# jinbeizame007/pytorch-r2d2-DPG

Hardware: NVIDIA H100
Metric: learner sequence-steps/sec (batch x seq_len) (higher is better)
Workload: dtype bf16x3 (fp32 operands split into bf16 hi+lo, three tensor-core passes, fp32 accumulate: ~16-bit operands)

## Files before the change

pytorch-r2d2-dpg_b200/csrc/gemm.cu:

```cuda
#include "gemm.cuh"
#include "elementwise.cuh"

#include <stdlib.h>

namespace r2d2 {
namespace {

constexpr int BM = 128, BN = 64, BK = 32, GEMM_THREADS = 256;

template <int LAYOUT>
struct TileGeom {
  static constexpr bool A_KMAJOR = (LAYOUT != GEMM_TN);
  static constexpr int A_ROWS = A_KMAJOR ? BM : BK;
  static constexpr int A_COLS = A_KMAJOR ? BK : BM;
  static constexpr int A_LD = A_COLS + 8;
  static constexpr bool B_KMAJOR = (LAYOUT == GEMM_NT);
  static constexpr int B_ROWS = B_KMAJOR ? BN : BK;
  static constexpr int B_COLS = B_KMAJOR ? BK : BN;
  static constexpr int B_LD = B_COLS + 8;
  static constexpr int A_PLANE = A_ROWS * A_LD;
  static constexpr int B_PLANE = B_ROWS * B_LD;
  static constexpr int STAGE = 2 * A_PLANE + 2 * B_PLANE;
  static constexpr int SMEM_BYTES = 2 * STAGE * (int)sizeof(__nv_bfloat16);
  static constexpr int A_F4_PER_ROW = A_COLS / 4;
  static constexpr int B_F4_PER_ROW = B_COLS / 4;
  static constexpr int A_F4 = A_ROWS * A_COLS / 4 / GEMM_THREADS;
  static constexpr int B_F4 = B_ROWS * B_COLS / 4 / GEMM_THREADS;
};

__device__ __forceinline__ float4 guarded_load4(const float* __restrict__ base, long long ld, int row, int col,
                                                int row_lim, int col_lim, bool vec) {
  float4 v = make_float4(0.f, 0.f, 0.f, 0.f);
  if (row < row_lim && col < col_lim) {
    const float* p = base + (long long)row * ld + col;
    if (vec && col + 3 < col_lim) {
      v = __ldg(reinterpret_cast<const float4*>(p));
    } else {
      v.x = __ldg(p);
      if (col + 1 < col_lim) v.y = __ldg(p + 1);
      if (col + 2 < col_lim) v.z = __ldg(p + 2);
      if (col + 3 < col_lim) v.w = __ldg(p + 3);
    }
  }
  return v;
}

__device__ __forceinline__ void store_split4(__nv_bfloat16* hi_plane, __nv_bfloat16* lo_plane, int off, float4 v) {
  uint32_t h0, l0, h1, l1;
  split_pack2(v.x, v.y, h0, l0);
  split_pack2(v.z, v.w, h1, l1);
  *reinterpret_cast<uint2*>(hi_plane + off) = make_uint2(h0, h1);
  *reinterpret_cast<uint2*>(lo_plane + off) = make_uint2(l0, l1);
}

template <int LAYOUT>
__global__ void __launch_bounds__(GEMM_THREADS)
gemm_bf16x3_kernel(GemmParams p, int vecA, int vecB, int vecA2, int vecB2, long long c_split_stride) {
  using G = TileGeom<LAYOUT>;
  extern __shared__ __align__(16) unsigned char smem_raw[];
  __nv_bfloat16* smem = reinterpret_cast<__nv_bfloat16*>(smem_raw);

  const int tid = threadIdx.x, lane = tid & 31, warp = tid >> 5;
  const int wm = warp & 3, wn = warp >> 2;
  const int m0 = blockIdx.y * BM, n0 = blockIdx.x * BN;

  const int nk1 = (p.K + BK - 1) / BK;
  const int nk2 = (p.K2 + BK - 1) / BK;
  const int nk_total = nk1 + nk2;
  const int per_split = (nk_total + p.split_k - 1) / p.split_k;
  const int t_begin = blockIdx.z * per_split;
  const int t_end = min(nk_total, t_begin + per_split);
  if (t_begin >= t_end) return;

  float acc[2][4][4];
#pragma unroll
  for (int i = 0; i < 2; ++i)
#pragma unroll
    for (int j = 0; j < 4; ++j)
#pragma unroll
      for (int e = 0; e < 4; ++e) acc[i][j][e] = 0.f;

  float4 ra[G::A_F4], rb[G::B_F4];

  auto load_tile = [&](int t) {
    const float* Ap; const float* Bp; long long lda, ldb; int k0, klim; bool va, vb;
    if (t < nk1) { Ap = p.A; Bp = p.B; lda = p.lda; ldb = p.ldb; k0 = t * BK; klim = p.K; va = vecA; vb = vecB; }
    else { Ap = p.A2; Bp = p.B2; lda = p.lda2; ldb = p.ldb2; k0 = (t - nk1) * BK; klim = p.K2; va = vecA2; vb = vecB2; }
#pragma unroll
    for (int i = 0; i < G::A_F4; ++i) {
      int q = tid + i * GEMM_THREADS;
      int r = q / G::A_F4_PER_ROW, c = (q % G::A_F4_PER_ROW) * 4;
      if (G::A_KMAJOR) ra[i] = guarded_load4(Ap, lda, m0 + r, k0 + c, p.M, klim, va);
      else             ra[i] = guarded_load4(Ap, lda, k0 + r, m0 + c, klim, p.M, va);
    }
#pragma unroll
    for (int i = 0; i < G::B_F4; ++i) {
      int q = tid + i * GEMM_THREADS;
      int r = q / G::B_F4_PER_ROW, c = (q % G::B_F4_PER_ROW) * 4;
      if (G::B_KMAJOR) rb[i] = guarded_load4(Bp, ldb, n0 + r, k0 + c, p.N, klim, vb);
      else             rb[i] = guarded_load4(Bp, ldb, k0 + r, n0 + c, klim, p.N, vb);
    }
  };

  auto store_tile = [&](int buf) {
    __nv_bfloat16* a_hi = smem + buf * G::STAGE;
    __nv_bfloat16* a_lo = a_hi + G::A_PLANE;
    __nv_bfloat16* b_hi = a_lo + G::A_PLANE;
    __nv_bfloat16* b_lo = b_hi + G::B_PLANE;
#pragma unroll
    for (int i = 0; i < G::A_F4; ++i) {
      int q = tid + i * GEMM_THREADS;
      int r = q / G::A_F4_PER_ROW, c = (q % G::A_F4_PER_ROW) * 4;
      store_split4(a_hi, a_lo, r * G::A_LD + c, ra[i]);
    }
#pragma unroll
    for (int i = 0; i < G::B_F4; ++i) {
      int q = tid + i * GEMM_THREADS;
      int r = q / G::B_F4_PER_ROW, c = (q % G::B_F4_PER_ROW) * 4;
      store_split4(b_hi, b_lo, r * G::B_LD + c, rb[i]);
    }
  };

  auto compute_tile = [&](int buf) {
    const __nv_bfloat16* a_hi = smem + buf * G::STAGE;
    const __nv_bfloat16* a_lo = a_hi + G::A_PLANE;
    const __nv_bfloat16* b_hi = a_lo + G::A_PLANE;
    const __nv_bfloat16* b_lo = b_hi + G::B_PLANE;
    const int j = lane >> 3, r = lane & 7;
#pragma unroll
    for (int kk = 0; kk < BK; kk += 16) {
      uint32_t fa_hi[2][4], fa_lo[2][4], fb_hi[4][2], fb_lo[4][2];
#pragma unroll
      for (int i = 0; i < 2; ++i) {
        if (G::A_KMAJOR) {
          int off = (wm * 32 + i * 16 + (j & 1) * 8 + r) * G::A_LD + kk + (j >> 1) * 8;
          ldmatrix_x4(fa_hi[i], a_hi + off);
          ldmatrix_x4(fa_lo[i], a_lo + off);
        } else {
          int off = (kk + (j >> 1) * 8 + r) * G::A_LD + wm * 32 + i * 16 + (j & 1) * 8;
          ldmatrix_x4_trans(fa_hi[i], a_hi + off);
          ldmatrix_x4_trans(fa_lo[i], a_lo + off);
        }
      }
#pragma unroll
      for (int pj = 0; pj < 2; ++pj) {
        uint32_t th[4], tl[4];
        if (G::B_KMAJOR) {
          int off = (wn * 32 + pj * 16 + (j >> 1) * 8 + r) * G::B_LD + kk + (j & 1) * 8;
          ldmatrix_x4(th, b_hi + off);
          ldmatrix_x4(tl, b_lo + off);
        } else {
          int off = (kk + (j & 1) * 8 + r) * G::B_LD + wn * 32 + pj * 16 + (j >> 1) * 8;
          ldmatrix_x4_trans(th, b_hi + off);
          ldmatrix_x4_trans(tl, b_lo + off);
        }
        fb_hi[2 * pj][0] = th[0]; fb_hi[2 * pj][1] = th[1]; fb_hi[2 * pj + 1][0] = th[2]; fb_hi[2 * pj + 1][1] = th[3];
        fb_lo[2 * pj][0] = tl[0]; fb_lo[2 * pj][1] = tl[1]; fb_lo[2 * pj + 1][0] = tl[2]; fb_lo[2 * pj + 1][1] = tl[3];
      }
#pragma unroll
      for (int i = 0; i < 2; ++i)
#pragma unroll
        for (int jn = 0; jn < 4; ++jn) {
          mma_bf16_16816(acc[i][jn], fa_lo[i], fb_hi[jn]);
          mma_bf16_16816(acc[i][jn], fa_hi[i], fb_lo[jn]);
          mma_bf16_16816(acc[i][jn], fa_hi[i], fb_hi[jn]);
        }
    }
  };

  load_tile(t_begin);
  store_tile(0);
  __syncthreads();
  for (int t = t_begin; t < t_end; ++t) {
    const int buf = (t - t_begin) & 1;
    if (t + 1 < t_end) load_tile(t + 1);
    compute_tile(buf);
    if (t + 1 < t_end) store_tile(buf ^ 1);
    __syncthreads();
  }

  const int g = lane >> 2, c = lane & 3;
  float* const C = p.C + (long long)blockIdx.z * c_split_stride;
  const bool vec_c = ((reinterpret_cast<uintptr_t>(C) & 7) == 0) && (p.ldc % 2 == 0);
#pragma unroll
  for (int i = 0; i < 2; ++i) {
#pragma unroll
    for (int jn = 0; jn < 4; ++jn) {
      const int col = n0 + wn * 32 + jn * 8 + 2 * c;
#pragma unroll
      for (int h = 0; h < 2; ++h) {
        const int row = m0 + wm * 32 + i * 16 + g + h * 8;
        if (row >= p.M || col >= p.N) continue;
        float v0 = acc[i][jn][2 * h], v1 = acc[i][jn][2 * h + 1];
        const bool has1 = (col + 1 < p.N);
        if (p.bias) { v0 += __ldg(p.bias + col); if (has1) v1 += __ldg(p.bias + col + 1); }
        if (p.epilogue == EPI_TANH) { v0 = tanhf(v0); v1 = tanhf(v1); }
        else if (p.epilogue == EPI_MUL_DTANH) {
          const float* z = p.Z + (long long)row * p.ldz + col;
          float z0 = z[0]; v0 *= (1.f - z0 * z0);
          if (has1) { float z1 = z[1]; v1 *= (1.f - z1 * z1); }
        } else if (p.epilogue == EPI_ADD_Z) {
          const float* z = p.Z + (long long)row * p.ldz + col;
          v0 += z[0];
          if (has1) v1 += z[1];
        }
        float* cp = C + (long long)row * p.ldc + col;
        if (vec_c && has1) {
          *reinterpret_cast<float2*>(cp) = make_float2(v0, v1);
        } else {
          cp[0] = v0;
          if (has1) cp[1] = v1;
        }
      }
    }
  }
}

template <int LAYOUT>
int launch_gemm(const GemmParams& p, cudaStream_t stream) {
  using G = TileGeom<LAYOUT>;
  static PerDeviceOnce once;
  if (once.need()) {
    R2D2_CUDA_TRY(cudaFuncSetAttribute(gemm_bf16x3_kernel<LAYOUT>, cudaFuncAttributeMaxDynamicSharedMemorySize,
                                       G::SMEM_BYTES));
  }
  auto aligned = [](const float* ptr, long long ld) {
    return ptr != nullptr && ((reinterpret_cast<uintptr_t>(ptr) & 15) == 0) && (ld % 4 == 0);
  };
  GemmParams q = p;
  int slices = 1;
  if (p.split_k > 1) {
    const int nk = ceil_div(p.K, BK) + ceil_div(p.K2, BK), per_split = ceil_div(nk, p.split_k);
    slices = ceil_div(nk, per_split);
    R2D2_TRY(partials_scratch((size_t)slices * p.M * p.N, stream, &q.C));
    q.ldc = p.N;
  }
  dim3 grid(ceil_div(p.N, BN), ceil_div(p.M, BM), slices);
  gemm_bf16x3_kernel<LAYOUT><<<grid, GEMM_THREADS, G::SMEM_BYTES, stream>>>(
      q, aligned(p.A, p.lda), aligned(p.B, p.ldb), aligned(p.A2, p.lda2), aligned(p.B2, p.ldb2), (long long)p.M * p.N);
  count_launch();
  R2D2_CUDA_TRY(cudaGetLastError());
  if (p.split_k > 1) return add_partials(q.C, slices, p.M, p.N, p.C, p.ldc, nullptr, stream);
  return R2D2_OK;
}

}

static int g_gemm_impl = -1;
void gemm_set_impl(int impl) { g_gemm_impl = impl ? 1 : 0; }
int gemm_get_impl() {
  if (g_gemm_impl < 0) {
    const char* e = getenv("R2D2_GEMM_IMPL");
    g_gemm_impl = (e && (e[0] == 'm' || e[0] == '0')) ? 0 : 1;
  }
  return g_gemm_impl;
}

static int g_skinny_mma = 1;
void gemm_set_impl_skinny_mma(int on) { g_skinny_mma = on ? 1 : 0; }
int gemm_get_impl_skinny_mma() { return g_skinny_mma; }

bool gemm_supports_bias2(int M, int N, int K) {
  const bool skinny = (K < 64) || (N < 32) || (M < 32);
  return gemm_get_impl() == 1 && !(skinny && gemm_get_impl_skinny_mma());
}

bool gemm_emits_operand_image(int M, int N, int K_total) {
  if (gemm_get_impl() != 1 || N <= 32 || N % 32 != 0) return false;
  if (gemm_get_impl_skinny_mma() && K_total <= 32) return true;
  const bool skinny = (K_total < 64) || (M < 32);
  return !(skinny && gemm_get_impl_skinny_mma());
}

int gemm_suggest_split_k(int M, int N, int K) {
  const bool skinny = (K < 64) || (N < 32) || (M < 32);
  if (gemm_get_impl() == 1 && !(skinny && g_skinny_mma)) return gemm_tc_suggest_split_k(M, N, K);
  long long tiles = (long long)ceil_div(M, BM) * ceil_div(N, BN);
  int k_tiles = ceil_div(K, BK);
  if (tiles >= num_sms() || k_tiles < 16) return 1;
  int want = (int)ceil_div_ll(2 * num_sms(), tiles);
  int max_by_k = k_tiles / 8;
  int s = want < max_by_k ? want : max_by_k;
  if (s < 1) s = 1;
  if (s > 128) s = 128;
  return s;
}

static int gemm_f32_dispatch(const GemmParams& p, GemmLayout layout, cudaStream_t stream, bool* colsums_done);

int gemm_f32(const GemmParams& p, GemmLayout layout, cudaStream_t stream) {
  R2D2_REQUIRE((!p.colsum_a && !p.colsum_b) || layout == GEMM_TN, "column sums ride on TN products only");
  bool colsums_done = false;
  R2D2_TRY(gemm_f32_dispatch(p, layout, stream, &colsums_done));
  if (!colsums_done) {
    if (p.colsum_a) R2D2_TRY(colsum(p.A, p.lda, p.K, p.M, p.colsum_a, nullptr, stream));
    if (p.colsum_b) R2D2_TRY(colsum(p.B, p.ldb, p.K, p.N, p.colsum_b, nullptr, stream));
  }
  return R2D2_OK;
}

static int gemm_f32_dispatch(const GemmParams& p, GemmLayout layout, cudaStream_t stream, bool* colsums_done) {
  R2D2_REQUIRE((p.A || p.A_img) && (p.B || p.B_img) && p.C, "null operand");
  if (p.A_img || p.B_img) {
    R2D2_REQUIRE(p.K2 == 0, "packed A with a second K segment");
    return gemm_f32_tc(p, layout, stream);
  }
  R2D2_REQUIRE(p.M > 0 && p.N > 0 && p.K > 0, "empty problem");
  R2D2_REQUIRE(p.split_k >= 1, "split_k");
  R2D2_REQUIRE(p.split_k == 1 || (p.epilogue == EPI_NONE && p.bias == nullptr), "split-K supports no epilogue");
  R2D2_REQUIRE(p.K2 == 0 || layout == GEMM_NT, "second K segment only for NT");
  R2D2_REQUIRE(p.K2 == 0 || (p.A2 && p.B2), "segment 2 operands");
  R2D2_REQUIRE((p.epilogue != EPI_MUL_DTANH && p.epilogue != EPI_ADD_Z) || p.Z, "epilogue needs Z");
  R2D2_REQUIRE(ceil_div(p.M, BM) <= 65535, "M too large for grid.y");
  const bool skinny = (p.K + p.K2 < 64) || (p.N < 32) || (p.M < 32);
  if (gemm_get_impl() == 1 && gemm_get_impl_skinny_mma()) {
    bool handled = false;
    R2D2_TRY(gemm_thin_try(p, layout, stream, &handled));
    if (handled) { *colsums_done = true; return R2D2_OK; }
  }
  R2D2_REQUIRE(!p.bias2 || gemm_supports_bias2(p.M, p.N, p.K + p.K2), "bias2 needs the wgmma path (gemm_supports_bias2)");
  R2D2_REQUIRE((!p.C_img_k && !p.C_img_mn) || (layout == GEMM_NT && gemm_emits_operand_image(p.M, p.N, p.K + p.K2)),
               "C_img_* is produced by the small-K streaming kernel and the wgmma epilogue only (see gemm_emits_operand_image)");
  if (gemm_get_impl() == 1 && !(skinny && gemm_get_impl_skinny_mma())) return gemm_f32_tc(p, layout, stream);
  switch (layout) {
    case GEMM_NT: return launch_gemm<GEMM_NT>(p, stream);
    case GEMM_NN: return launch_gemm<GEMM_NN>(p, stream);
    case GEMM_TN: return launch_gemm<GEMM_TN>(p, stream);
  }
  set_last_error("bad gemm layout");
  return R2D2_ERR_ARG;
}

}
```

pytorch-r2d2-dpg_b200/csrc/gemm.cuh:

```cuda
#pragma once
#include "common.cuh"

namespace r2d2 {

enum GemmLayout : int {
  GEMM_NT = 0,
  GEMM_NN = 1,
  GEMM_TN = 2
};

enum GemmEpilogue : int {
  EPI_NONE = 0,
  EPI_TANH = 1,
  EPI_MUL_DTANH = 2,
  EPI_ADD_Z = 3
};

struct GemmParams {
  const float* A = nullptr;  long long lda = 0;
  const float* B = nullptr;  long long ldb = 0;
  const float* A2 = nullptr; long long lda2 = 0;
  const float* B2 = nullptr; long long ldb2 = 0;
  int K2 = 0;
  float* C = nullptr;        long long ldc = 0;
  int M = 0, N = 0, K = 0;
  const float* bias = nullptr;
  const float* bias2 = nullptr;
  const float* Z = nullptr;  long long ldz = 0;
  int epilogue = EPI_NONE;
  int split_k = 1;
  const unsigned char* A_img = nullptr;
  unsigned char* C_img_k = nullptr;
  unsigned char* C_img_mn = nullptr;
  const unsigned char* B_img = nullptr;
  float* colsum_a = nullptr;
  float* colsum_b = nullptr;
  int reuse_packed_a = 0;
};

int gemm_f32(const GemmParams& p, GemmLayout layout, cudaStream_t stream);
bool gemm_emits_operand_image(int M, int N, int K_total);
bool gemm_supports_bias2(int M, int N, int K);
int gemm_suggest_split_k(int M, int N, int K);

void gemm_set_impl(int impl);
int gemm_get_impl();
void gemm_set_impl_skinny_mma(int on);
int gemm_get_impl_skinny_mma();
int gemm_f32_tc(const GemmParams& p, GemmLayout layout, cudaStream_t stream);
int gemm_thin_try(const GemmParams& p, GemmLayout layout, cudaStream_t stream, bool* handled);
int gemm_tc_suggest_split_k(int M, int N, int K);

}
```

pytorch-r2d2-dpg_b200/csrc/gemm_tc.cu:

```cuda
#include <stdlib.h>

#include <map>
#include <mutex>
#include <utility>

#include "elementwise.cuh"
#include "gemm.cuh"
#include "sm90.cuh"

namespace r2d2 {
namespace {

constexpr int TBM = 128, TBN = 128, TBK = 32;
constexpr int PLANE_BYTES = 128 * TBK * 2;
constexpr int TILE_BYTES = 2 * PLANE_BYTES;
constexpr int PACKED_GEMM_THREADS = 288;
constexpr int CTAS_PER_SM = 2;
constexpr int STAGES = 3;
constexpr int STAGE_BYTES = 2 * TILE_BYTES;
constexpr int OFF_BARS = STAGES * STAGE_BYTES;
constexpr int PACKED_SMEM = OFF_BARS + 128;

template <bool MN_MAJOR>
__global__ void __launch_bounds__(256) pack_operand_kernel(const float* __restrict__ src, long long ld, int mn_lim,
                                                           int k_lim, int k_tiles_total, int k_tile_offset, int vec,
                                                           unsigned char* __restrict__ dst) {
  const int mn0 = blockIdx.y * 128, k0 = blockIdx.x * TBK;
  unsigned char* tile = dst + ((size_t)blockIdx.y * k_tiles_total + k_tile_offset + blockIdx.x) * TILE_BYTES;
#pragma unroll
  for (int g = 0; g < 2; ++g) {
    const int id = threadIdx.x + g * 256;
    int row, col, row_lim, col_lim;
    if (MN_MAJOR) { row = k0 + 8 * (id >> 7) + (id & 7); col = mn0 + 8 * ((id >> 3) & 15); row_lim = k_lim; col_lim = mn_lim; }
    else          { row = mn0 + 8 * (id >> 5) + (id & 7); col = k0 + 8 * ((id >> 3) & 3);  row_lim = mn_lim; col_lim = k_lim; }
    float v[8];
#pragma unroll
    for (int i = 0; i < 8; ++i) v[i] = 0.f;
    if (row < row_lim && col < col_lim) {
      const float* p = src + (long long)row * ld + col;
      if (vec && col + 7 < col_lim) {
        const float4 a = __ldg(reinterpret_cast<const float4*>(p)), b = __ldg(reinterpret_cast<const float4*>(p + 4));
        v[0] = a.x; v[1] = a.y; v[2] = a.z; v[3] = a.w; v[4] = b.x; v[5] = b.y; v[6] = b.z; v[7] = b.w;
      } else {
#pragma unroll
        for (int i = 0; i < 8; ++i) if (col + i < col_lim) v[i] = __ldg(p + i);
      }
    }
    uint4 h, l;
    split_pack2(v[0], v[1], h.x, l.x);
    split_pack2(v[2], v[3], h.y, l.y);
    split_pack2(v[4], v[5], h.z, l.z);
    split_pack2(v[6], v[7], h.w, l.w);
    *reinterpret_cast<uint4*>(tile + id * 16) = h;
    *reinterpret_cast<uint4*>(tile + PLANE_BYTES + id * 16) = l;
  }
}

__device__ __forceinline__ void mbar_wait_spin(uint64_t* bar, uint32_t parity) {
  while (!sm90::mbar_try_wait(bar, parity)) {}
}

struct PackedGemmParams {
  const unsigned char* pa;
  const unsigned char* pb;
  int k_tiles;
  float* C; long long ldc;
  int M, N;
  const float* bias;
  const float* bias2;
  const float* Z; long long ldz;
  int epilogue, split_k;
  long long c_split_stride;
  unsigned char* c_img_k;
  unsigned char* c_img_mn;
};

template <bool A_MN, bool B_MN>
__global__ void __launch_bounds__(PACKED_GEMM_THREADS, CTAS_PER_SM) gemm_packed_kernel(PackedGemmParams p) {
  extern __shared__ __align__(128) unsigned char smem[];
  uint64_t* full = reinterpret_cast<uint64_t*>(smem + OFF_BARS);
  uint64_t* empty = full + STAGES;

  const int tid = threadIdx.x, lane = tid & 31;
  const int wg = __shfl_sync(0xffffffffu, tid >> 7, 0);
  const int m_tile = blockIdx.y, n_tile = blockIdx.x;
  const int m0 = m_tile * TBM, n0 = n_tile * TBN;
  const int per_split = (p.k_tiles + p.split_k - 1) / p.split_k;
  const int t_begin = blockIdx.z * per_split;
  const int t_end = min(p.k_tiles, t_begin + per_split);
  if (t_begin >= t_end) return;
  const int n_tiles = t_end - t_begin;

  if (tid == 0) {
    for (int s = 0; s < STAGES; ++s) { sm90::mbar_init(&full[s], 1); sm90::mbar_init(&empty[s], 2); }
    asm volatile("fence.mbarrier_init.release.cluster;" ::: "memory");
  }
  __syncthreads();

  if (wg == 2) {
    if (sm90::elect_one()) {
      const unsigned char* a_src = p.pa + ((size_t)m_tile * p.k_tiles + t_begin) * TILE_BYTES;
      const unsigned char* b_src = p.pb + ((size_t)n_tile * p.k_tiles + t_begin) * TILE_BYTES;
      const uint32_t smem_base = sm90::smem_u32(smem);
      for (int i = 0; i < n_tiles; ++i) {
        const int s = i % STAGES;
        mbar_wait_spin(&empty[s], ((i / STAGES) & 1) ^ 1);
        const uint32_t bar = sm90::smem_u32(&full[s]);
        sm90::mbar_arrive_expect_tx(&full[s], 2 * TILE_BYTES);
        sm90::bulk_copy_g2s(smem_base + s * STAGE_BYTES, a_src + (size_t)i * TILE_BYTES, TILE_BYTES, bar);
        sm90::bulk_copy_g2s(smem_base + s * STAGE_BYTES + TILE_BYTES, b_src + (size_t)i * TILE_BYTES, TILE_BYTES, bar);
      }
    }
    return;
  }

  const int half = wg, t = tid & 127;
  float acc[64];
#pragma unroll
  for (int i = 0; i < 64; ++i) acc[i] = 0.f;
  const uint32_t a_lbo = A_MN ? 2048 : 128, a_sbo = A_MN ? 128 : 512;
  const uint32_t b_lbo = B_MN ? 2048 : 128, b_sbo = B_MN ? 128 : 512;
  const uint32_t a_ks = A_MN ? 4096 : 256, b_ks = B_MN ? 4096 : 256;
  const uint32_t a_half = half * 8 * a_sbo;
  const uint32_t smem_base = sm90::smem_u32(smem);
  for (int i = 0; i < n_tiles; ++i) {
    const int s = i % STAGES;
    mbar_wait_spin(&full[s], (i / STAGES) & 1);
    const uint32_t sa = smem_base + s * STAGE_BYTES + a_half, sb = smem_base + s * STAGE_BYTES + TILE_BYTES;
    sm90::fence_regs(acc);
    sm90::wgmma_fence();
#pragma unroll
    for (int ks = 0; ks < TBK / 16; ++ks) {
      const uint64_t a_hi = sm90::make_smem_desc(sa + ks * a_ks, a_lbo, a_sbo);
      const uint64_t a_lo = sm90::make_smem_desc(sa + ks * a_ks + PLANE_BYTES, a_lbo, a_sbo);
      const uint64_t b_hi = sm90::make_smem_desc(sb + ks * b_ks, b_lbo, b_sbo);
      const uint64_t b_lo = sm90::make_smem_desc(sb + ks * b_ks + PLANE_BYTES, b_lbo, b_sbo);
      sm90::wgmma_m64n128k16_bf16<A_MN, B_MN>(acc, a_lo, b_hi);
      sm90::wgmma_m64n128k16_bf16<A_MN, B_MN>(acc, a_hi, b_lo);
      sm90::wgmma_m64n128k16_bf16<A_MN, B_MN>(acc, a_hi, b_hi);
    }
    sm90::wgmma_commit();
    sm90::wgmma_wait<1>();
    sm90::fence_regs(acc);
    __syncwarp();
    if (i > 0 && t == 0) sm90::mbar_arrive(&empty[(i - 1) % STAGES]);
  }
  sm90::wgmma_wait<0>();
  sm90::fence_regs(acc);
  __syncwarp();
  if (t == 0) sm90::mbar_arrive(&empty[(n_tiles - 1) % STAGES]);

  const int r_base = m0 + half * 64 + 16 * (t >> 5) + (lane >> 2);
  const int c_off = 2 * (lane & 3);
  float* const C = p.C + (long long)blockIdx.z * p.c_split_stride;
  const bool vec_c = ((reinterpret_cast<uintptr_t>(C) & 7) == 0) && (p.ldc % 2 == 0);
  const bool img = p.c_img_k != nullptr || p.c_img_mn != nullptr;
#pragma unroll
  for (int j = 0; j < TBN / 8; ++j) {
    const int col = n0 + 8 * j + c_off;
    const bool c0ok = col < p.N, c1ok = col + 1 < p.N;
    float b0 = 0.f, b1 = 0.f;
    if (p.bias) {
      if (c0ok) b0 = __ldg(p.bias + col) + (p.bias2 ? __ldg(p.bias2 + col) : 0.f);
      if (c1ok) b1 = __ldg(p.bias + col + 1) + (p.bias2 ? __ldg(p.bias2 + col + 1) : 0.f);
    }
#pragma unroll
    for (int h = 0; h < 2; ++h) {
      const int row = r_base + 8 * h;
      float v0 = acc[4 * j + 2 * h] + b0, v1 = acc[4 * j + 2 * h + 1] + b1;
      if (img) {
        const bool ok = row < p.M && c0ok;
        if (ok) {
          if (p.epilogue == EPI_TANH) { v0 = tanhf(v0); v1 = tanhf(v1); }
          *reinterpret_cast<float2*>(p.C + (long long)row * p.ldc + col) = make_float2(v0, v1);
        } else {
          v0 = v1 = 0.f;
        }
        uint32_t hw, lw;
        split_pack2(v0, v1, hw, lw);
        const int q0 = lane & ~3;
        const uint4 hi = make_uint4(__shfl_sync(0xffffffffu, hw, q0), __shfl_sync(0xffffffffu, hw, q0 + 1),
                                    __shfl_sync(0xffffffffu, hw, q0 + 2), __shfl_sync(0xffffffffu, hw, q0 + 3));
        const uint4 lo = make_uint4(__shfl_sync(0xffffffffu, lw, q0), __shfl_sync(0xffffffffu, lw, q0 + 1),
                                    __shfl_sync(0xffffffffu, lw, q0 + 2), __shfl_sync(0xffffffffu, lw, q0 + 3));
        const int cg = n0 + 8 * j;
        if ((lane & 3) == 0 && cg < p.N && row < ((p.M + 31) & ~31)) {
          if (p.c_img_k && row < p.M) {
            unsigned char* d = p.c_img_k + ((size_t)(row >> 7) * (p.N >> 5) + (cg >> 5)) * TILE_BYTES +
                               ((((row & 127) >> 3) * 32) + ((cg & 31) >> 3) * 8 + (row & 7)) * 16;
            *reinterpret_cast<uint4*>(d) = hi;
            *reinterpret_cast<uint4*>(d + PLANE_BYTES) = lo;
          }
          if (p.c_img_mn) {
            unsigned char* d = p.c_img_mn + ((size_t)(cg >> 7) * ((p.M + 31) >> 5) + (row >> 5)) * TILE_BYTES +
                               ((((row & 31) >> 3) * 128) + ((cg & 127) >> 3) * 8 + (row & 7)) * 16;
            *reinterpret_cast<uint4*>(d) = hi;
            *reinterpret_cast<uint4*>(d + PLANE_BYTES) = lo;
          }
        }
        continue;
      }
      if (row >= p.M || !c0ok) continue;
      if (p.epilogue == EPI_TANH) {
        v0 = tanhf(v0); v1 = tanhf(v1);
      } else if (p.epilogue == EPI_MUL_DTANH || p.epilogue == EPI_ADD_Z) {
        const float* z = p.Z + (long long)row * p.ldz + col;
        const float z0 = z[0], z1 = c1ok ? z[1] : 0.f;
        if (p.epilogue == EPI_MUL_DTANH) { v0 *= 1.f - z0 * z0; v1 *= 1.f - z1 * z1; }
        else { v0 += z0; v1 += z1; }
      }
      float* cp = C + (long long)row * p.ldc + col;
      if (vec_c && c1ok) {
        *reinterpret_cast<float2*>(cp) = make_float2(v0, v1);
      } else {
        cp[0] = v0;
        if (c1ok) cp[1] = v1;
      }
    }
  }
}

struct Scratch { unsigned char* ptr = nullptr; size_t bytes = 0; };
struct LastPackedA { const float* ptr = nullptr; long long ld = 0; int mn = 0, k = 0, mn_major = 0, k_tiles = 0; };
struct StreamScratch { Scratch a, b; LastPackedA last_a; };
std::mutex g_scratch_mutex;
std::map<std::pair<int, cudaStream_t>, StreamScratch> g_scratch;

int scratch_for(cudaStream_t stream, StreamScratch** out) {
  int dev = 0;
  R2D2_CUDA_TRY(cudaGetDevice(&dev));
  std::lock_guard<std::mutex> lock(g_scratch_mutex);
  *out = &g_scratch[std::make_pair(dev, stream)];
  return R2D2_OK;
}

int ensure_scratch(Scratch& s, size_t bytes) {
  if (s.bytes >= bytes) return R2D2_OK;
  if (s.ptr) { R2D2_CUDA_TRY(cudaDeviceSynchronize()); R2D2_CUDA_TRY(cudaFree(s.ptr)); s.ptr = nullptr; s.bytes = 0; }
  const size_t want = bytes + bytes / 4 + (1u << 20);
  R2D2_CUDA_TRY(cudaMalloc(&s.ptr, want));
  s.bytes = want;
  return R2D2_OK;
}

int launch_pack(const float* src, long long ld, int mn_lim, int k_lim, bool mn_major, int mn_tiles, int k_tiles_total,
                int k_tile_offset, unsigned char* dst, cudaStream_t stream) {
  const int vec = (((reinterpret_cast<uintptr_t>(src) & 15) == 0) && (ld % 4 == 0)) ? 1 : 0;
  dim3 grid(ceil_div(k_lim, TBK), mn_tiles);
  if (mn_major) pack_operand_kernel<true><<<grid, 256, 0, stream>>>(src, ld, mn_lim, k_lim, k_tiles_total, k_tile_offset, vec, dst);
  else          pack_operand_kernel<false><<<grid, 256, 0, stream>>>(src, ld, mn_lim, k_lim, k_tiles_total, k_tile_offset, vec, dst);
  count_launch();
  R2D2_CUDA_TRY(cudaGetLastError());
  return R2D2_OK;
}

}

int gemm_tc_suggest_split_k(int M, int N, int K) {
  long long tiles = (long long)ceil_div(M, TBM) * ceil_div(N, TBN);
  int k_tiles = ceil_div(K, TBK);
  if (tiles >= num_sms() || k_tiles < 16) return 1;
  int want = (int)ceil_div_ll(2 * num_sms(), tiles);
  int max_by_k = k_tiles / 8;
  int s = want < max_by_k ? want : max_by_k;
  if (s < 1) s = 1;
  if (s > 256) s = 256;
  return s;
}

template <bool A_MN, bool B_MN>
int launch_packed(const PackedGemmParams& q, int m_tiles, int n_tiles, int slices, cudaStream_t stream) {
  static PerDeviceOnce once;
  if (once.need()) {
    R2D2_CUDA_TRY(cudaFuncSetAttribute(gemm_packed_kernel<A_MN, B_MN>, cudaFuncAttributeMaxDynamicSharedMemorySize,
                                       PACKED_SMEM));
  }
  dim3 grid(n_tiles, m_tiles, slices);
  gemm_packed_kernel<A_MN, B_MN><<<grid, PACKED_GEMM_THREADS, PACKED_SMEM, stream>>>(q);
  count_launch();
  R2D2_CUDA_TRY(cudaGetLastError());
  return R2D2_OK;
}

int gemm_f32_tc(const GemmParams& p, GemmLayout layout, cudaStream_t stream) {
  const bool a_mn = (layout == GEMM_TN), b_mn = (layout != GEMM_NT);
  const int m_tiles = ceil_div(p.M, TBM), n_tiles = ceil_div(p.N, TBN);
  const int kt1 = ceil_div(p.K, TBK), kt2 = p.K2 > 0 ? ceil_div(p.K2, TBK) : 0;
  const int k_tiles = kt1 + kt2;
  R2D2_REQUIRE(m_tiles <= 65535, "M too large for grid.y");
  StreamScratch* sc = nullptr;
  R2D2_TRY(scratch_for(stream, &sc));
  Scratch& g_pack_a = sc->a;
  Scratch& g_pack_b = sc->b;
  LastPackedA& last_a = sc->last_a;
  if (!p.A_img) R2D2_TRY(ensure_scratch(g_pack_a, (size_t)m_tiles * k_tiles * TILE_BYTES));
  if (!p.B_img) R2D2_TRY(ensure_scratch(g_pack_b, (size_t)n_tiles * k_tiles * TILE_BYTES));
  const bool reuse = p.reuse_packed_a && kt2 == 0 && last_a.ptr == p.A && last_a.ld == p.lda && last_a.mn == p.M &&
                     last_a.k == p.K && last_a.mn_major == (a_mn ? 1 : 0) && last_a.k_tiles == k_tiles;
  if (!p.A_img) {
    if (!reuse) R2D2_TRY(launch_pack(p.A, p.lda, p.M, p.K, a_mn, m_tiles, k_tiles, 0, g_pack_a.ptr, stream));
    last_a = LastPackedA{kt2 ? nullptr : p.A, p.lda, p.M, p.K, a_mn ? 1 : 0, k_tiles};
  }
  if (!p.B_img) R2D2_TRY(launch_pack(p.B, p.ldb, p.N, p.K, b_mn, n_tiles, k_tiles, 0, g_pack_b.ptr, stream));
  if (kt2) {
    R2D2_REQUIRE(!p.A_img && !p.B_img, "packed operand with a second K segment");
    R2D2_TRY(launch_pack(p.A2, p.lda2, p.M, p.K2, a_mn, m_tiles, k_tiles, kt1, g_pack_a.ptr, stream));
    R2D2_TRY(launch_pack(p.B2, p.ldb2, p.N, p.K2, b_mn, n_tiles, k_tiles, kt1, g_pack_b.ptr, stream));
  }
  PackedGemmParams q;
  q.pa = p.A_img ? p.A_img : g_pack_a.ptr; q.pb = p.B_img ? p.B_img : g_pack_b.ptr; q.k_tiles = k_tiles; q.C = p.C; q.ldc = p.ldc; q.M = p.M; q.N = p.N;
  q.bias = p.bias; q.bias2 = p.bias ? p.bias2 : nullptr; q.Z = p.Z; q.ldz = p.ldz; q.epilogue = p.epilogue; q.split_k = p.split_k;
  q.c_img_k = p.C_img_k; q.c_img_mn = p.C_img_mn;
  q.c_split_stride = 0;
  int slices = 1;
  if (p.split_k > 1) {
    slices = ceil_div(k_tiles, ceil_div(k_tiles, p.split_k));
    R2D2_TRY(partials_scratch((size_t)slices * p.M * p.N, stream, &q.C));
    q.ldc = p.N;
    q.c_split_stride = (long long)p.M * p.N;
  }
  if (p.C_img_k || p.C_img_mn) {
    R2D2_REQUIRE(p.N % 32 == 0 && p.split_k == 1 && (p.epilogue == EPI_NONE || p.epilogue == EPI_TANH) &&
                     (reinterpret_cast<uintptr_t>(p.C) & 7) == 0 && p.ldc % 2 == 0,
                 "operand image from the wgmma epilogue: N % 32 == 0, no split-K, bias / tanh epilogue, 8-byte aligned C");
  }
  if (a_mn) R2D2_TRY((launch_packed<true, true>(q, m_tiles, n_tiles, slices, stream)));
  else if (b_mn) R2D2_TRY((launch_packed<false, true>(q, m_tiles, n_tiles, slices, stream)));
  else R2D2_TRY((launch_packed<false, false>(q, m_tiles, n_tiles, slices, stream)));
  if (p.split_k > 1) return add_partials(q.C, slices, p.M, p.N, p.C, p.ldc, nullptr, stream);
  return R2D2_OK;
}

}
```

pytorch-r2d2-dpg_b200/csrc/net.cu:

```cuda
#include "net.cuh"

#include "elementwise.cuh"
#include "gemm.cuh"
#include "lstm_scan.cuh"

namespace r2d2 {

static size_t align64(size_t n) { return (n + 63) & ~(size_t)63; }
static size_t pad_to(size_t n, size_t m) { return (n + m - 1) / m * m; }

size_t ChainWs::floats(const NetShape& s, int T, int B, int repeat) {
  const size_t H = s.hidden, A = s.act, S = (size_t)T * repeat, TB = (size_t)T * B;
  size_t n = 0;
  n += align64(TB * H);
  n += align64(TB * 4 * H);
  if (repeat > 1) n += align64(S * B * 4 * H);
  n += 2 * align64((S + 1) * B * H);
  n += align64(TB * H);
  n += align64(TB * H);
  n += 2 * align64(TB * A);
  n += align64(4 * H);
  size_t sc = lstm_scan_fwd_scratch_floats(B, s.hidden);
  const size_t sb = lstm_scan_bwd_scratch_floats(B, s.hidden);
  if (sb > sc) sc = sb;
  n += align64(sc + 64);
  n += align64(pad_to(TB, 128) * H);
  return n;
}

ChainWs ChainWs::carve(float* base, const NetShape& s, int T, int B, int repeat) {
  const size_t H = s.hidden, A = s.act, S = (size_t)T * repeat, TB = (size_t)T * B;
  ChainWs w;
  float* p = base;
  auto take = [&](size_t n) { float* r = p; p += align64(n); return r; };
  w.z1 = take(TB * H);
  w.gin = take(TB * 4 * H);
  w.gates = (repeat > 1) ? take(S * B * 4 * H) : w.gin;
  w.hs = take((S + 1) * B * H);
  w.cs = take((S + 1) * B * H);
  w.head_in = take(TB * H);
  w.dh_head = take(TB * H);
  w.head_out = take(TB * A);
  w.d_pre = take(TB * A);
  w.bias_sum = take(4 * H);
  size_t sc = lstm_scan_fwd_scratch_floats(B, s.hidden);
  const size_t sb = lstm_scan_bwd_scratch_floats(B, s.hidden);
  if (sb > sc) sc = sb;
  w.scratch = take(sc + 64);
  w.img_k = reinterpret_cast<unsigned char*>(take(pad_to(TB, 128) * H));
  return w;
}

int net_forward(const NetShape& s, const NetParams& P, const ChainWs& ws, const float* obs, const float* act,
                const float* h0, const float* c0, int T, int B, int repeat, cudaStream_t stream) {
  R2D2_TRY(net_forward_inputs(s, P, ws, obs, act, T, B, stream));
  return net_forward_scan(s, P, ws, h0, c0, T, B, repeat, stream);
}

int net_forward_inputs(const NetShape& s, const NetParams& P, const ChainWs& ws, const float* obs, const float* act,
                       int T, int B, cudaStream_t stream) {
  const int H = s.hidden, O = s.obs, A = s.act, I = s.in_features();
  const int M = T * B;
  R2D2_REQUIRE(!s.critic || act != nullptr, "critic needs actions");
  bool z1_img = false;
  {
    GemmParams g;
    g.A = obs; g.lda = O; g.B = P.w1; g.ldb = I; g.K = O;
    if (s.critic) { g.A2 = act; g.lda2 = A; g.B2 = P.w1 + O; g.ldb2 = I; g.K2 = A; }
    g.C = ws.z1; g.ldc = H; g.M = M; g.N = H; g.bias = P.b1; g.epilogue = EPI_TANH;
    z1_img = ws.img_k != nullptr && gemm_emits_operand_image(M, H, I);
    if (z1_img) g.C_img_k = ws.img_k;
    R2D2_TRY(gemm_f32(g, GEMM_NT, stream));
  }
  const bool two_bias = gemm_supports_bias2(M, 4 * H, H);
  if (!two_bias) R2D2_TRY(add_vec(P.bih, P.bhh, ws.bias_sum, 4 * H, stream));
  {
    GemmParams g;
    g.A = ws.z1; g.lda = H; g.B = P.wih; g.ldb = H; g.K = H;
    g.C = ws.gin; g.ldc = 4 * H; g.M = M; g.N = 4 * H;
    if (two_bias) { g.bias = P.bih; g.bias2 = P.bhh; } else g.bias = ws.bias_sum;
    if (z1_img) g.A_img = ws.img_k;
    R2D2_TRY(gemm_f32(g, GEMM_NT, stream));
  }
  return R2D2_OK;
}

int net_forward_scan(const NetShape& s, const NetParams& P, const ChainWs& ws, const float* h0, const float* c0, int T,
                     int B, int repeat, cudaStream_t stream) {
  const int H = s.hidden;
  ScanFwdParams sp;
  sp.gin = ws.gin; sp.whh = P.whh; sp.h0 = h0; sp.c0 = c0;
  sp.gates = ws.gates; sp.hs = ws.hs; sp.cs = ws.cs;
  sp.head_in = s.critic ? nullptr : ws.head_in;
  sp.T = T; sp.B = B; sp.H = H; sp.repeat = repeat; sp.scratch = ws.scratch;
  sp.no_save = ws.inference_only ? 1 : 0;
  return lstm_scan_forward(sp, stream);
}

static const float* head_input(const NetShape& s, const ChainWs& ws, int first_row, int B) {
  return s.critic ? ws.hs + (size_t)(1 + first_row) * B * s.hidden : ws.head_in + (size_t)first_row * B * s.hidden;
}

int net_head_forward(const NetShape& s, const NetParams& P, const ChainWs& ws, int first_row, int T, int B,
                     int repeat, float* out, long long ldo, cudaStream_t stream) {
  R2D2_REQUIRE(!s.critic || repeat == 1, "critic chains run one cell step per row");
  R2D2_REQUIRE(first_row >= 0 && first_row < T, "head_first_row");
  GemmParams g;
  g.A = head_input(s, ws, first_row, B); g.lda = s.hidden;
  g.B = P.w3; g.ldb = s.hidden; g.K = s.hidden;
  g.C = out; g.ldc = ldo; g.M = (T - first_row) * B; g.N = s.act; g.bias = P.b3;
  g.epilogue = s.critic ? EPI_NONE : EPI_TANH;
  return gemm_f32(g, GEMM_NT, stream);
}

int net_backward(const NetShape& s, const NetParams& P, const NetParams* G, const ChainWs& ws, const float* obs,
                 const float* act, const float* d_pre, int first_row, int T, int B, int repeat, float* d_act,
                 const float* dact_z, cudaStream_t stream) {
  const int H = s.hidden, O = s.obs, A = s.act, I = s.in_features();
  const int S = T * repeat, M = T * B, Mh = (T - first_row) * B;
  R2D2_REQUIRE(!s.critic || repeat == 1, "critic chains run one cell step per row");
  const float* hin = head_input(s, ws, first_row, B);
  if (G) {
    GemmParams g;
    g.A = d_pre; g.lda = A; g.B = hin; g.ldb = H; g.K = Mh;
    g.C = G->w3; g.ldc = H; g.M = A; g.N = H; g.split_k = gemm_suggest_split_k(A, H, Mh);
    g.colsum_a = G->b3;
    R2D2_TRY(gemm_f32(g, GEMM_TN, stream));
  }
  {
    GemmParams g;
    g.A = d_pre; g.lda = A; g.B = P.w3; g.ldb = H; g.K = A;
    g.C = ws.dh_head; g.ldc = H; g.M = Mh; g.N = H;
    if (!s.critic) { g.Z = hin; g.ldz = H; g.epilogue = EPI_MUL_DTANH; }
    R2D2_TRY(gemm_f32(g, GEMM_NN, stream));
  }
  float* dgin = (repeat > 1) ? ws.gin : ws.gates;
  {
    ScanBwdParams bp;
    bp.gates = ws.gates; bp.hs = ws.hs; bp.cs = ws.cs; bp.whh = P.whh;
    bp.dh_head = ws.dh_head; bp.head_first_step = first_row * repeat;
    bp.dgates = ws.gates; bp.dgin = dgin;
    bp.T = T; bp.B = B; bp.H = H; bp.repeat = repeat; bp.scratch = ws.scratch;
    if (G) { bp.dbias = G->bih; bp.dbias2 = G->bhh; }
    R2D2_TRY(lstm_scan_backward(bp, stream));
  }
  if (G) {
    {
      GemmParams g;
      g.A = ws.gates; g.lda = 4 * H; g.B = ws.hs; g.ldb = H; g.K = S * B;
      g.C = G->whh; g.ldc = H; g.M = 4 * H; g.N = H; g.split_k = gemm_suggest_split_k(4 * H, H, S * B);
      R2D2_TRY(gemm_f32(g, GEMM_TN, stream));
    }
    {
      GemmParams g;
      g.A = dgin; g.lda = 4 * H; g.B = ws.z1; g.ldb = H; g.K = M;
      g.C = G->wih; g.ldc = H; g.M = 4 * H; g.N = H; g.split_k = gemm_suggest_split_k(4 * H, H, M);
      g.reuse_packed_a = (repeat == 1);
      R2D2_TRY(gemm_f32(g, GEMM_TN, stream));
    }
  }
  {
    GemmParams g;
    g.A = dgin; g.lda = 4 * H; g.B = P.wih; g.ldb = H; g.K = 4 * H;
    g.C = ws.z1; g.ldc = H; g.M = M; g.N = H; g.Z = ws.z1; g.ldz = H; g.epilogue = EPI_MUL_DTANH;
    R2D2_TRY(gemm_f32(g, GEMM_NN, stream));
  }
  if (G) {
    GemmParams g;
    g.A = ws.z1; g.lda = H; g.B = obs; g.ldb = O; g.K = M;
    g.C = G->w1; g.ldc = I; g.M = H; g.N = O; g.split_k = gemm_suggest_split_k(H, O, M);
    g.colsum_a = G->b1;
    R2D2_TRY(gemm_f32(g, GEMM_TN, stream));
    if (s.critic) {
      GemmParams g2 = g;
      g2.colsum_a = nullptr;
      g2.B = act; g2.ldb = A; g2.C = G->w1 + O; g2.N = A; g2.split_k = gemm_suggest_split_k(H, A, M);
      R2D2_TRY(gemm_f32(g2, GEMM_TN, stream));
    }
  }
  if (d_act) {
    R2D2_REQUIRE(s.critic, "d_act only for the critic");
    GemmParams g;
    g.A = ws.z1; g.lda = H; g.B = P.w1 + O; g.ldb = I; g.K = H;
    g.C = d_act; g.ldc = A; g.M = M; g.N = A;
    if (dact_z) { g.Z = dact_z; g.ldz = A; g.epilogue = EPI_MUL_DTANH; }
    R2D2_TRY(gemm_f32(g, GEMM_NN, stream));
  }
  return R2D2_OK;
}

}
```

Before: 1.240 million.

## Gather A tiles from previously packed transposed image instead of repacking

When the NN GEMM's A operand (dgin) was just packed MN-major for the preceding TN weight-gradient GEMM, the producer warp now gathers 512-byte sub-blocks from that existing packed image via per-lane bulk copies instead of launching a new pack kernel. This removes a pack kernel launch and its global read/write of the A matrix. In exchange, the producer issues many small bulk copies per stage instead of one, and packed-A cache state is now invalidated on non-tensor-core paths to keep the reuse correct.

```diff
diff --git a/pytorch-r2d2-dpg_b200/csrc/gemm.cu b/pytorch-r2d2-dpg_b200/csrc/gemm.cu
--- a/pytorch-r2d2-dpg_b200/csrc/gemm.cu
+++ b/pytorch-r2d2-dpg_b200/csrc/gemm.cu
@@ -316,12 +316,13 @@
   if (gemm_get_impl() == 1 && gemm_get_impl_skinny_mma()) {
     bool handled = false;
     R2D2_TRY(gemm_thin_try(p, layout, stream, &handled));
-    if (handled) { *colsums_done = true; return R2D2_OK; }
+    if (handled) { gemm_tc_forget_packed_a(stream); *colsums_done = true; return R2D2_OK; }
   }
   R2D2_REQUIRE(!p.bias2 || gemm_supports_bias2(p.M, p.N, p.K + p.K2), "bias2 needs the wgmma path (gemm_supports_bias2)");
   R2D2_REQUIRE((!p.C_img_k && !p.C_img_mn) || (layout == GEMM_NT && gemm_emits_operand_image(p.M, p.N, p.K + p.K2)),
                "C_img_* is produced by the small-K streaming kernel and the wgmma epilogue only (see gemm_emits_operand_image)");
   if (gemm_get_impl() == 1 && !(skinny && gemm_get_impl_skinny_mma())) return gemm_f32_tc(p, layout, stream);
+  gemm_tc_forget_packed_a(stream);
   switch (layout) {
     case GEMM_NT: return launch_gemm<GEMM_NT>(p, stream);
     case GEMM_NN: return launch_gemm<GEMM_NN>(p, stream);
diff --git a/pytorch-r2d2-dpg_b200/csrc/gemm.cuh b/pytorch-r2d2-dpg_b200/csrc/gemm.cuh
--- a/pytorch-r2d2-dpg_b200/csrc/gemm.cuh
+++ b/pytorch-r2d2-dpg_b200/csrc/gemm.cuh
@@ -50,5 +50,6 @@
 int gemm_f32_tc(const GemmParams& p, GemmLayout layout, cudaStream_t stream);
 int gemm_thin_try(const GemmParams& p, GemmLayout layout, cudaStream_t stream, bool* handled);
 int gemm_tc_suggest_split_k(int M, int N, int K);
+void gemm_tc_forget_packed_a(cudaStream_t stream);
 
 }
diff --git a/pytorch-r2d2-dpg_b200/csrc/gemm_tc.cu b/pytorch-r2d2-dpg_b200/csrc/gemm_tc.cu
--- a/pytorch-r2d2-dpg_b200/csrc/gemm_tc.cu
+++ b/pytorch-r2d2-dpg_b200/csrc/gemm_tc.cu
@@ -73,6 +73,7 @@
   long long c_split_stride;
   unsigned char* c_img_k;
   unsigned char* c_img_mn;
+  int a_gather, a_img_k_tiles;
 };
 
 template <bool A_MN, bool B_MN>
@@ -98,18 +99,26 @@
   __syncthreads();
 
   if (wg == 2) {
-    if (sm90::elect_one()) {
-      const unsigned char* a_src = p.pa + ((size_t)m_tile * p.k_tiles + t_begin) * TILE_BYTES;
-      const unsigned char* b_src = p.pb + ((size_t)n_tile * p.k_tiles + t_begin) * TILE_BYTES;
-      const uint32_t smem_base = sm90::smem_u32(smem);
-      for (int i = 0; i < n_tiles; ++i) {
-        const int s = i % STAGES;
-        mbar_wait_spin(&empty[s], ((i / STAGES) & 1) ^ 1);
-        const uint32_t bar = sm90::smem_u32(&full[s]);
-        sm90::mbar_arrive_expect_tx(&full[s], 2 * TILE_BYTES);
-        sm90::bulk_copy_g2s(smem_base + s * STAGE_BYTES, a_src + (size_t)i * TILE_BYTES, TILE_BYTES, bar);
-        sm90::bulk_copy_g2s(smem_base + s * STAGE_BYTES + TILE_BYTES, b_src + (size_t)i * TILE_BYTES, TILE_BYTES, bar);
-      }
+    const uint32_t smem_base = sm90::smem_u32(smem);
+    const unsigned char* a_src = p.pa + ((size_t)m_tile * p.k_tiles + t_begin) * TILE_BYTES;
+    const unsigned char* b_src = p.pb + ((size_t)n_tile * p.k_tiles + t_begin) * TILE_BYTES;
+    const int groups = p.a_gather ? min(16, (32 * p.a_img_k_tiles - m0) / 8) : 16;
+    const int g = lane & 15, plane = lane >> 4, row = m0 + 8 * g;
+    for (int i = 0; i < n_tiles; ++i) {
+      const int s = i % STAGES, t = t_begin + i;
+      mbar_wait_spin(&empty[s], ((i / STAGES) & 1) ^ 1);
+      const uint32_t bar = sm90::smem_u32(&full[s]), da = smem_base + s * STAGE_BYTES;
+      if (lane == 0) {
+        sm90::mbar_arrive_expect_tx(&full[s], TILE_BYTES + (p.a_gather ? groups * 2 * 512 : TILE_BYTES));
+        sm90::bulk_copy_g2s(da + TILE_BYTES, b_src + (size_t)i * TILE_BYTES, TILE_BYTES, bar);
+        if (!p.a_gather) sm90::bulk_copy_g2s(da, a_src + (size_t)i * TILE_BYTES, TILE_BYTES, bar);
+      }
+      if (p.a_gather && g < groups) {
+        const unsigned char* src = p.pa + ((size_t)(t >> 2) * p.a_img_k_tiles + (row >> 5)) * TILE_BYTES +
+                                   plane * PLANE_BYTES + ((row & 31) >> 3) * 2048 + (t & 3) * 512;
+        sm90::bulk_copy_g2s(da + plane * PLANE_BYTES + g * 512, src, 512, bar);
+      }
+      __syncwarp();
     }
     return;
   }
@@ -256,6 +265,11 @@
 
 }
 
+void gemm_tc_forget_packed_a(cudaStream_t stream) {
+  StreamScratch* sc = nullptr;
+  if (scratch_for(stream, &sc) == R2D2_OK) sc->last_a = LastPackedA{};
+}
+
 int gemm_tc_suggest_split_k(int M, int N, int K) {
   long long tiles = (long long)ceil_div(M, TBM) * ceil_div(N, TBN);
   int k_tiles = ceil_div(K, TBK);
@@ -293,11 +307,13 @@
   Scratch& g_pack_a = sc->a;
   Scratch& g_pack_b = sc->b;
   LastPackedA& last_a = sc->last_a;
-  if (!p.A_img) R2D2_TRY(ensure_scratch(g_pack_a, (size_t)m_tiles * k_tiles * TILE_BYTES));
   if (!p.B_img) R2D2_TRY(ensure_scratch(g_pack_b, (size_t)n_tiles * k_tiles * TILE_BYTES));
   const bool reuse = p.reuse_packed_a && kt2 == 0 && last_a.ptr == p.A && last_a.ld == p.lda && last_a.mn == p.M &&
                      last_a.k == p.K && last_a.mn_major == (a_mn ? 1 : 0) && last_a.k_tiles == k_tiles;
-  if (!p.A_img) {
+  const bool gather = p.reuse_packed_a && !p.A_img && !a_mn && kt2 == 0 && p.K % TBK == 0 && last_a.ptr == p.A &&
+                      last_a.ld == p.lda && last_a.mn == p.K && last_a.k == p.M && last_a.mn_major == 1;
+  if (!p.A_img && !gather) {
+    R2D2_TRY(ensure_scratch(g_pack_a, (size_t)m_tiles * k_tiles * TILE_BYTES));
     if (!reuse) R2D2_TRY(launch_pack(p.A, p.lda, p.M, p.K, a_mn, m_tiles, k_tiles, 0, g_pack_a.ptr, stream));
     last_a = LastPackedA{kt2 ? nullptr : p.A, p.lda, p.M, p.K, a_mn ? 1 : 0, k_tiles};
   }
@@ -312,6 +328,8 @@
   q.bias = p.bias; q.bias2 = p.bias ? p.bias2 : nullptr; q.Z = p.Z; q.ldz = p.ldz; q.epilogue = p.epilogue; q.split_k = p.split_k;
   q.c_img_k = p.C_img_k; q.c_img_mn = p.C_img_mn;
   q.c_split_stride = 0;
+  q.a_gather = gather ? 1 : 0;
+  q.a_img_k_tiles = gather ? last_a.k_tiles : 0;
   int slices = 1;
   if (p.split_k > 1) {
     slices = ceil_div(k_tiles, ceil_div(k_tiles, p.split_k));
diff --git a/pytorch-r2d2-dpg_b200/csrc/net.cu b/pytorch-r2d2-dpg_b200/csrc/net.cu
--- a/pytorch-r2d2-dpg_b200/csrc/net.cu
+++ b/pytorch-r2d2-dpg_b200/csrc/net.cu
@@ -163,6 +163,7 @@
     GemmParams g;
     g.A = dgin; g.lda = 4 * H; g.B = P.wih; g.ldb = H; g.K = 4 * H;
     g.C = ws.z1; g.ldc = H; g.M = M; g.N = H; g.Z = ws.z1; g.ldz = H; g.epilogue = EPI_MUL_DTANH;
+    g.reuse_packed_a = (G != nullptr);
     R2D2_TRY(gemm_f32(g, GEMM_NN, stream));
   }
   if (G) {
```

Measured after the change: 1.245 million (median of 6 runs). No clear change (+0.4%).
